# open-mmlab/Live2Diff

Hardware: AMD Instinct MI355X
Metric: frames/sec @512×512, 2 denoise steps; per-step latency; 1/2/4/8 GPU (higher is better)
Workload: dtype f16; 1 GPU; BASELINE configs[1]: 512x512 image (64x64 latent), 2 denoise steps, KV window L=16 (8 sink + 8 rolling), SD-1.5 UNet widths + Live2Diff temporal attention, one independent stream per GPU; plan_launches=433, hipgraph=False, device=AMD Radeon Graphics (gfx950:sramecc+:xnack-, 256 CUs), output_finite=True, default_workload=True

## Files before the change

### live2diff_amd/csrc/flash_attn.hip

```cpp
#include "common.h"

struct FAArgs {
    const h16 *q, *k, *vt;
    h16 *out;
    int B, H, d, Tq, Tk, ldq, ldk, ldvt, ldo;
    long long sq, sk, svt, so;
};

template <int D>
struct FACfg {
    static constexpr int DQK = ((D + 31) / 32) * 32;
    static constexpr int KK = DQK / 32;
    static constexpr int D16 = (D + 15) / 16;
    static constexpr int KROW = DQK + 16;
    static constexpr int VROW = 72;
    static constexpr int KCH = (64 * (DQK / 8)) / 256;
    static constexpr int VTOT = D16 * 16 * 8;
    static constexpr int VCH = (VTOT + 255) / 256;
    static constexpr int TILE_HALFS = 64 * KROW + D16 * 16 * VROW;
    static constexpr int NBUF = (TILE_HALFS * 2 * 2 <= 65536) ? 2 : 1;
    static constexpr bool ONES = (D % 16) != 0;
};

template <int D>
// ... 114 lines not shown
                mx = fmaxf(fmaxf(mx, fmaxf(sacc[ks][qs][0], sacc[ks][qs][1])), fmaxf(sacc[ks][qs][2], sacc[ks][qs][3]));
            mx = fmaxf(mx, __shfl_xor(mx, 16, 64));
            mx = fmaxf(mx, __shfl_xor(mx, 32, 64));
            if (__any((mx - mrow[qs]) * c2e > 8.0f)) {
                const float mnew = fmaxf(mrow[qs], mx);
                const float alpha = __builtin_amdgcn_exp2f((mrow[qs] - mnew) * c2e);
                mrow[qs] = mnew;
                lrow[qs] *= alpha;
#pragma unroll
                for (int ds = 0; ds < D16; ++ds) oacc[ds][qs] *= alpha;
            }
            const float mneg = -mrow[qs] * c2e;
            float psum = 0.f;
#pragma unroll
            for (int ks = 0; ks < 4; ++ks)
#pragma unroll
                for (int r = 0; r < 4; ++r) {
                    const float pv = __builtin_amdgcn_exp2f(fmaf(sacc[ks][qs][r], c2e, mneg));
                    if (!Cf::ONES) psum += pv;
                    pf[ks >> 1][qs][(ks & 1) * 4 + r] = (h16)pv;
                }
            if (!Cf::ONES) lrow[qs] += psum;
        }
#pragma unroll
        for (int c2 = 0; c2 < 2; ++c2)
#pragma unroll
            for (int ds = 0; ds < D16; ++ds) {
                const h16 *vr = Vs + (ds * 16 + li) * VROW + c2 * 32 + lg * 4;
                h16x4 lo = *reinterpret_cast<const h16x4 *>(vr);
                h16x4 hi = *reinterpret_cast<const h16x4 *>(vr + 16);
                h16x8 vf = __builtin_shufflevector(lo, hi, 0, 1, 2, 3, 4, 5, 6, 7);
#pragma unroll
                for (int qs = 0; qs < 2; ++qs)
                    oacc[ds][qs] = __builtin_amdgcn_mfma_f32_16x16x32_f16(vf, pf[c2][qs], oacc[ds][qs], 0, 0, 0);
            }
        if (NBUF == 2) {
            if (kt + 1 < nt) store_tiles(cur ^ 1);
            __syncthreads();
            cur ^= 1;
        } else {
            __syncthreads();
            if (kt + 1 < nt) store_tiles(0);
            __syncthreads();
        }
    }
#pragma unroll
    for (int qs = 0; qs < 2; ++qs) {
        float l;
        if (Cf::ONES) {
            l = __shfl(oacc[D / 16][qs][D % 4], ((D % 16) / 4) * 16 + li, 64);
        } else {
            l = lrow[qs];
            l += __shfl_xor(l, 16, 64);
            l += __shfl_xor(l, 32, 64);
        }
        const float inv = 1.0f / l;
        const int qr = q0 + qs * 16 + li;
        if (qr >= a.Tq) continue;
#pragma unroll
        for (int ds = 0; ds < D16; ++ds) {
            int dc = ds * 16 + lg * 4;
            if (dc >= D) continue;
            h16x4 o;
#pragma unroll
            for (int r = 0; r < 4; ++r) o[r] = (h16)(oacc[ds][qs][r] * inv);
            *reinterpret_cast<h16x4 *>(op + (long long)qr * a.ldo + dc) = o;
        }
    }
}

template <int D>
__global__ __launch_bounds__(256) void flash_attn_kernel(FAArgs a) { flash_attn_body<D>(a); }
template <int D>
__global__ __launch_bounds__(256) __attribute__((amdgpu_waves_per_eu(2))) void flash_attn_kernel_w2(FAArgs a) { flash_attn_body<D>(a); }

template <int D>
static void launch_fa(const FAArgs &a, hipStream_t s) {
    dim3 grid((a.Tq + 127) / 128, a.H, a.B);
    if (D <= 80) hipLaunchKernelGGL((flash_attn_kernel_w2<D>), grid, dim3(256), 0, s, a);
    else hipLaunchKernelGGL((flash_attn_kernel<D>), grid, dim3(256), 0, s, a);
}

int l2d_launch_flash_ring(const l2d_op *op, int qs, hipStream_t s);

int l2d_launch_flash_attn(const l2d_op *op, hipStream_t s) {
    FAArgs a;
    a.q = (const h16 *)op->p[0]; a.k = (const h16 *)op->p[1]; a.vt = (const h16 *)op->p[2]; a.out = (h16 *)op->p[3];
    a.B = op->i[0]; a.H = op->i[1]; a.d = op->i[2]; a.Tq = op->i[3]; a.Tk = op->i[4];
    a.ldq = op->i[5]; a.ldk = op->i[6]; a.ldvt = op->i[7]; a.ldo = op->i[8];
    a.sq = op->l[0]; a.sk = op->l[1]; a.svt = op->l[2]; a.so = op->l[3];
    if (!a.q || !a.k || !a.vt || !a.out || a.B <= 0 || a.H <= 0 || a.Tq <= 0 || a.Tk <= 0 || (a.ldq % 8) || (a.ldk % 8) ||
        (a.ldvt % 8) || (a.ldo % 4) || a.ldvt < ((a.Tk + 7) / 8) * 8) {
        l2d_set_error("flash_attn(tag %d): invalid arguments (B=%d H=%d d=%d Tq=%d Tk=%d ldvt=%d)", op->tag, a.B, a.H, a.d,
                      a.Tq, a.Tk, a.ldvt);
        return L2D_EINVAL;
    }
    const int variant = op->i[9];
    if (variant < 0 || variant > 4) {
        l2d_set_error("flash_attn(tag %d): unknown variant %d", op->tag, variant);
        return L2D_EINVAL;
    }
    const bool ring_ok = op->p[4] && (a.d % 8) == 0 && ((((uintptr_t)a.k) | ((uintptr_t)a.vt)) & 15) == 0 &&
                         ((a.sk | a.svt) % 8) == 0;
    if (variant >= 2 && !ring_ok) {
        l2d_set_error("flash_attn(tag %d): ring variant needs p4 = zero page, d %% 8 == 0 and 16-byte aligned K / V^T", op->tag);
        return L2D_EINVAL;
    }
    L2D_DRY_RETURN();
    if (variant != 1 && ring_ok) {
        int rc = l2d_launch_flash_ring(op, variant >= 2 ? variant : 0, s);
        if (rc != L2D_OK) {
            l2d_set_error("flash_attn(tag %d): unsupported head dim %d (built: 8,16,32,40,64,80,160)", op->tag, a.d);
            return rc;
        }
        return l2d_check_launch("flash_attn_ring", op->tag);
    }
    switch (a.d) {
        case 8: launch_fa<8>(a, s); break;
        case 16: launch_fa<16>(a, s); break;
        case 32: launch_fa<32>(a, s); break;
        case 40: launch_fa<40>(a, s); break;
        case 64: launch_fa<64>(a, s); break;
        case 80: launch_fa<80>(a, s); break;
        case 160: launch_fa<160>(a, s); break;
        default:
            l2d_set_error("flash_attn(tag %d): unsupported head dim %d (built: 8,16,32,40,64,80,160)", op->tag, a.d);
            return L2D_EINVAL;
    }
    return l2d_check_launch("flash_attn", op->tag);
}
```

### live2diff_amd/csrc/tattn.hip

```cpp
#include "tattn.h"

__device__ __forceinline__ float dot8(h16x8 a, h16x8 b) {
    float s = 0.f;
#pragma unroll
    for (int e = 0; e < 8; ++e) s += (float)a[e] * (float)b[e];
    return s;
}

template <int TP, int PB, int L, bool PV = true, int ABL = 0>
__global__ __launch_bounds__(TP *PB) void tattn_stream_kernel(TAttnArgs a) {
    constexpr int HG = TP / 8;
    constexpr int LP = L + 4;
    constexpr bool PRELOAD_V = PV && (L <= 24);
    extern __shared__ __attribute__((aligned(16))) float sp[];

    const int tid = threadIdx.x;
    const int p = tid / TP, cc = tid - p * TP;
    const long long NT = (long long)a.N * a.T;
    const long long pix = (long long)blockIdx.x * PB + p;
    const bool valid = pix < NT;
    const int n = valid ? (int)(pix / a.T) : 0;
    const long long t = valid ? pix - (long long)n * a.T : 0;
    const int C = a.C;
    const int u = (int)a.update_idx[n];
// ... 337 lines not shown
    int v = a.variant;
    if (v == 0) v = (L <= 16) ? 1 : 2;
    if (v == 1 && L <= 16)
        hipLaunchKernelGGL((tattn_stream_kernel<TP, PB, (L <= 16 ? L : 16)>), dim3(nb), dim3(TP * PB), lds, s, a);
#ifdef L2D_PROBES
    else if (v == 8 && L <= 16)
        hipLaunchKernelGGL((tattn_stream_kernel<TP, PB, (L <= 16 ? L : 16), true, 1>), dim3(nb), dim3(TP * PB), lds, s, a);
    else if (v == 9 && L <= 16)
        hipLaunchKernelGGL((tattn_stream_kernel<TP, PB, (L <= 16 ? L : 16), true, 2>), dim3(nb), dim3(TP * PB), lds, s, a);
    else if (v >= 10 && v <= 12 && L <= 16) {
        constexpr int LL = (L <= 16 ? L : 16);
        if (v == 10) hipLaunchKernelGGL((tattn_probe_kernel<TP, PB, LL, 0>), dim3(nb), dim3(TP * PB), 0, s, a);
        if (v == 11) hipLaunchKernelGGL((tattn_probe_kernel<TP, PB, LL, 1>), dim3(nb), dim3(TP * PB), 0, s, a);
        if (v == 12) hipLaunchKernelGGL((tattn_probe_kernel<TP, PB, LL, 2>), dim3(nb), dim3(TP * PB), 0, s, a);
    }
#else
    else if (v >= 8 && v <= 12) {
        l2d_set_error("tattn_stream: variants 8-12 are analysis probes (output is not attention); build with `make PROBES=1`");
        return L2D_EINVAL;
    }
#endif
    else if (v == 7 && L <= 16)
        hipLaunchKernelGGL((tattn_stream_lds_kernel<TP, PB, (L <= 16 ? L : 16)>), dim3(nb), dim3(TP * PB),
                           lds + (size_t)2 * L * TP * 8 * sizeof(h16), s, a);
    else if (v == 5 && L <= 16)
        hipLaunchKernelGGL((tattn_stream_kernel<TP, PB, (L <= 16 ? L : 16), false>), dim3(nb), dim3(TP * PB), lds, s, a);
    else if (v == 6 && L <= 16 && PB >= 2) {
        constexpr int PB2 = PB >= 2 ? PB / 2 : 1;
        int nb2 = (int)((NT + PB2 - 1) / PB2);
        hipLaunchKernelGGL((tattn_stream_kernel<TP, PB2, (L <= 16 ? L : 16)>), dim3(nb2), dim3(TP * PB2),
                           (size_t)TP * PB2 * (L + 4) * sizeof(float), s, a);
    }
    else if (v == 3)
        hipLaunchKernelGGL((tattn_stream_chunked_kernel<TP, PB, L, 4>), dim3(nb), dim3(TP * PB), lds, s, a);
    else if (v == 4 && L % 16 == 0)
        hipLaunchKernelGGL((tattn_stream_chunked_kernel<TP, PB, L, (L % 16 == 0 ? 16 : 4)>), dim3(nb), dim3(TP * PB), lds, s, a);
    else
        hipLaunchKernelGGL((tattn_stream_chunked_kernel<TP, PB, L, (L % 8 == 0 ? 8 : 4)>), dim3(nb), dim3(TP * PB), lds, s, a);
    return L2D_OK;
}

template <int TP, int PB>
static int launch_stream_l(const TAttnArgs &a, hipStream_t s) {
    switch (a.L) {
        case 12: return launch_stream_t<TP, PB, 12>(a, s);
        case 16: return launch_stream_t<TP, PB, 16>(a, s);
        case 24: return launch_stream_t<TP, PB, 24>(a, s);
        case 40: return launch_stream_t<TP, PB, 40>(a, s);
    }
    l2d_set_error("tattn_stream: unsupported window L=%d (built: 12,16,24,40)", a.L);
    return L2D_EINVAL;
}

static int tattn_common(const l2d_op *op, TAttnArgs &a, const char *what) {
    a.qkv = (const h16 *)op->p[0]; a.cache = (h16 *)op->p[1];
    a.q_pe = (const h16 *)op->p[2]; a.k_pe = (const h16 *)op->p[3]; a.v_pe = (const h16 *)op->p[4];
    a.pe_idx = (const long long *)op->p[5]; a.update_idx = (const long long *)op->p[6];
    a.bias = (const h16 *)op->p[7]; a.out = (h16 *)op->p[8];
    a.N = op->i[0]; a.T = op->i[1]; a.C = op->i[2]; a.L = op->i[3]; a.H = op->i[4]; a.variant = op->i[5];
#ifdef L2D_PROBES
    {
        extern unsigned long long *l2d_tattn_probe_ptr();
        a.probe = l2d_tattn_probe_ptr();
    }
#endif
    if (!a.qkv || !a.cache || !a.q_pe || !a.k_pe || !a.v_pe || !a.out || a.N <= 0 || a.T <= 0 || a.H != 8 ||
        (a.C % 64) || a.L <= 0) {
        l2d_set_error("%s(tag %d): invalid arguments (N=%d T=%d C=%d L=%d H=%d; need H=8, C%%64==0)", what, op->tag, a.N,
                      a.T, a.C, a.L, a.H);
        return L2D_EINVAL;
    }
    return L2D_OK;
}

int l2d_launch_tattn_stream(const l2d_op *op, hipStream_t s) {
    TAttnArgs a;
    int rc = tattn_common(op, a, "tattn_stream");
    if (rc) return rc;
    if (!a.pe_idx || !a.update_idx || !a.bias) {
        l2d_set_error("tattn_stream(tag %d): pe_idx/update_idx/bias missing", op->tag);
        return L2D_EINVAL;
    }
    L2D_DRY_RETURN();
    if (a.variant == 13 || (a.variant == 0 && l2d_tattn_ring_ok(a, op->p[9]))) {
        if (!l2d_tattn_ring_ok(a, op->p[9])) {
            l2d_set_error("tattn_stream(tag %d): ring variant needs C in {320,640,1280}, L in {12,16,24,40}, T %% 8 == 0, p9 = zero page", op->tag);
            return L2D_EINVAL;
        }
        rc = l2d_launch_tattn_ring(a, op->p[9], s);
        if (rc) return rc;
        return l2d_check_launch("tattn_stream_ring", op->tag);
    }
    switch (a.C) {
        case 64: rc = launch_stream_l<8, 32>(a, s); break;
        case 128: rc = launch_stream_l<16, 16>(a, s); break;
        case 256: rc = launch_stream_l<32, 8>(a, s); break;
        case 320: rc = launch_stream_l<40, 8>(a, s); break;
        case 640: rc = launch_stream_l<80, 4>(a, s); break;
        case 1280: rc = launch_stream_l<160, 2>(a, s); break;
        default:
            l2d_set_error("tattn_stream(tag %d): unsupported C=%d (built: 64,128,256,320,640,1280)", op->tag, a.C);
            return L2D_EINVAL;
    }
    if (rc) return rc;
    return l2d_check_launch("tattn_stream", op->tag);
}

template <int TP, int PB, int F>
__global__ __launch_bounds__(TP *PB) void tattn_warmup_kernel(TAttnArgs a) {
    constexpr int HG = TP / 8;
    constexpr int LP = F * F + 4;
    extern __shared__ __attribute__((aligned(16))) float sp[];
    const int tid = threadIdx.x;
    const int p = tid / TP, cc = tid - p * TP;
    const long long t = (long long)blockIdx.x * PB + p;
    const bool valid = t < a.T;
    const int C = a.C, L = a.L;
    h16x8 q[F], k[F], v[F];
#pragma unroll
    for (int f = 0; f < F; ++f) {
        q[f] = k[f] = v[f] = l2d_zero8();
        if (valid) {
            const h16 *src = a.qkv + ((long long)f * a.T + t) * 3 * C + cc * 8;
            q[f] = l2d_ld8(src);
            k[f] = l2d_ld8(src + C);
            v[f] = l2d_ld8(src + 2 * C);
            l2d_st8(a.cache + ((0LL * a.T + t) * L + f) * C + cc * 8, k[f]);
            l2d_st8(a.cache + ((1LL * a.T + t) * L + f) * C + cc * 8, v[f]);
        }
        q[f] = q[f] + l2d_ld8(a.q_pe + (long long)f * C + cc * 8);
        k[f] = k[f] + l2d_ld8(a.k_pe + (long long)f * C + cc * 8);
        v[f] = v[f] + l2d_ld8(a.v_pe + (long long)f * C + cc * 8);
    }
    float *row = sp + (long long)tid * LP;
#pragma unroll
    for (int fq = 0; fq < F; ++fq)
#pragma unroll
        for (int fk = 0; fk < F; fk += 4)
            *reinterpret_cast<f32x4 *>(row + fq * F + fk) =
                (f32x4){dot8(q[fq], k[fk]), dot8(q[fq], k[fk + 1]), dot8(q[fq], k[fk + 2]), dot8(q[fq], k[fk + 3])};
    __syncthreads();
    const int gs = p * TP + (cc / HG) * HG;
    const float scale = rsqrtf((float)(C / a.H));
#pragma unroll
    for (int fq = 0; fq < F; ++fq) {
        float s[F];
#pragma unroll
        for (int fk = 0; fk < F; ++fk) s[fk] = 0.f;
        for (int j = 0; j < HG; ++j) {
            const float *r = sp + (long long)(gs + j) * LP + fq * F;
#pragma unroll
            for (int fk = 0; fk < F; fk += 4) {
                f32x4 x = *reinterpret_cast<const f32x4 *>(r + fk);
                s[fk] += x[0]; s[fk + 1] += x[1]; s[fk + 2] += x[2]; s[fk + 3] += x[3];
            }
        }
        float mx = -3.0e38f;
#pragma unroll
        for (int fk = 0; fk < F; ++fk) { s[fk] *= scale; mx = fmaxf(mx, s[fk]); }
        float den = 0.f;
#pragma unroll
        for (int fk = 0; fk < F; ++fk) { s[fk] = __expf(s[fk] - mx); den += s[fk]; }
        const float inv = 1.0f / den;
        float o[8];
#pragma unroll
        for (int e = 0; e < 8; ++e) o[e] = 0.f;
#pragma unroll
// ... 48 lines not shown
```

### live2diff_amd/csrc/tattn_ring.hip

```cpp
#include <stdlib.h>

#include "tattn.h"

#define L2D_GPTR(p) ((__attribute__((address_space(1))) const void *)(p))
#define L2D_LPTR(p) ((__attribute__((address_space(3))) void *)(p))

typedef unsigned int u32x4 __attribute__((ext_vector_type(4)));

#ifdef L2D_PROBES
static unsigned long long *g_tattn_probe = nullptr;
extern "C" void l2d_tattn_set_probe(void *p) { g_tattn_probe = (unsigned long long *)p; }
unsigned long long *l2d_tattn_probe_ptr() { return g_tattn_probe; }
#define TR_STAMP(gi, s, i)                                                                                          \
    do {                                                                                                            \
        if (a.probe && (gi) == 1 && ((s) == 1 || (s) == NSTG / 2 + 1) && (threadIdx.x & 63) == 0)                    \
            a.probe[(((unsigned long long)blockIdx.x * 16 + (threadIdx.x >> 6)) * 2 + ((s) == 1 ? 0 : 1)) * 8 + (i)] = \
                __builtin_readcyclecounter();                                                                       \
    } while (0)
#else
#define TR_STAMP(gi, s, i) do { } while (0)
#endif

__device__ __forceinline__ float ring_dot8(h16x8 a, h16x8 b) {
    float s = 0.f;
// ... 106 lines not shown
        h16x8 q8 = qn;
        if (gi == 0) q8 = l2d_ld8(qkv_b + qoff);
        q8 = q8 + qpe;
        h16 *ku = kbase + (long long)gi * (PB * L * C) + u * C;
        float sc[L];
        float o[8];
#pragma unroll
        for (int e = 0; e < 8; ++e) o[e] = 0.f;
#pragma unroll
        for (int s = 0; s < NSTG; ++s) {
            TR_STAMP(gi, s, 0);
            if (total - 1 - it >= NS - 2) asm volatile("s_waitcnt vmcnt(%0) lgkmcnt(0)" ::"n"((NS - 2) * LPS) : "memory");
            else asm volatile("s_waitcnt vmcnt(0) lgkmcnt(0)" ::: "memory");
            TR_STAMP(gi, s, 1);
            __builtin_amdgcn_s_barrier();
            TR_STAMP(gi, s, 2);
            const bool refill = it_issue < total;
            if (refill) issue();
            TR_STAMP(gi, s, 3);
            const h16 *st = ring + cs_slot * STAGE_H + tid * 8;
            if (s < NSTG / 2) {
#pragma unroll
                for (int r = 0; r < R; ++r) {
                    const int l = s * R + r;
                    h16x8 kk = l2d_ld8(st + r * NT * 8);
                    if (l == u) l2d_st8(ku + coff, kk);
                    kk = kk + l2d_ld8(kpt + l * 320);
                    sc[l] = ring_dot8(q8, kk);
                }
                if (s == NSTG / 2 - 1) {
#pragma unroll
                    for (int l = 0; l < L; l += 4) *reinterpret_cast<f32x4 *>(row + l) = (f32x4){sc[l], sc[l + 1], sc[l + 2], sc[l + 3]};
                    asm volatile("s_waitcnt lgkmcnt(0)" ::: "memory");
                    __builtin_amdgcn_s_barrier();
#pragma unroll
                    for (int l = 0; l < L; ++l) sc[l] = 0.f;
#pragma unroll 2
                    for (int j = 0; j < HG; ++j) {
                        const float *rr = sp + (gs + j) * LP;
#pragma unroll
                        for (int l = 0; l < L; l += 4) {
                            f32x4 x = *reinterpret_cast<const f32x4 *>(rr + l);
                            sc[l] += x[0]; sc[l + 1] += x[1]; sc[l + 2] += x[2]; sc[l + 3] += x[3];
                        }
                    }
                    float mx = -3.0e38f;
#pragma unroll
                    for (int l = 0; l < L; l += 4) {
                        const f32x4 b4 = *reinterpret_cast<const f32x4 *>(blds + l);
#pragma unroll
                        for (int e = 0; e < 4; ++e) { sc[l + e] = sc[l + e] * scale + b4[e]; mx = fmaxf(mx, sc[l + e]); }
                    }
                    float den = 0.f;
#pragma unroll
                    for (int l = 0; l < L; ++l) { sc[l] = __expf(sc[l] - mx); den += sc[l]; }
                    const float inv = 1.0f / den;
#pragma unroll
                    for (int l = 0; l < L; ++l) sc[l] *= inv;
                }
            } else {
                if (s == NSTG / 2 && gi + 1 < ng)
                    qn = l2d_ld8(qkv_b + (long long)(gi + 1) * (PB * 3 * C) + qoff);
#pragma unroll
                for (int r = 0; r < R; ++r) {
                    const int l = (s - NSTG / 2) * R + r;
                    h16x8 vv = l2d_ld8(st + r * NT * 8);
                    if (l == u) l2d_st8(ku + slab + coff, vv);
                    vv = vv + l2d_ld8(vpt + l * 320);
                    ring_axpy8(o, sc[l], vv);
                }
            }
            TR_STAMP(gi, s, 4);
            ++it;
            cs_slot = (cs_slot + 1 == NS) ? 0 : cs_slot + 1;
        }
        h16x8 ov;
#pragma unroll
        for (int e = 0; e < 8; ++e) ov[e] = (h16)o[e];
        l2d_st8(out_b + (long long)gi * (PB * C) + ooff, ov);
    }
}
#endif

template <int HG, int L, int R, int NS>
__global__ __launch_bounds__(384) void tattn_stream_ringlw_kernel(TAttnArgs a, const h16 *zero, int gpb, int groups_per_unit) {
    constexpr int PB = 8, TP = 40, NT = TP * PB, NSTG = 2 * L / R, LPSL = 5 * R;
    constexpr int STAGE_H = R * PB * TP * 8;
    constexpr int LP = L + 4;
    static_assert((NS - 2) * LPSL < 64 && L % 4 == 0 && L % R == 0, "geometry");
    extern __shared__ __attribute__((aligned(16))) unsigned char ring_raw[];
    h16 *ring = reinterpret_cast<h16 *>(ring_raw);
    float *sp = reinterpret_cast<float *>(ring_raw + (size_t)NS * STAGE_H * sizeof(h16));
    float *blds = sp + NT * LP;
    h16 *kpl = reinterpret_cast<h16 *>(blds + L);
    h16 *vpl = kpl + L * 320;

    const int tid = threadIdx.x;
    const int wave = __builtin_amdgcn_readfirstlane(tid >> 6);
    const int C = a.C, CH = C / 320;
    const int bpu = (groups_per_unit + gpb - 1) / gpb;
    const int unit = __builtin_amdgcn_readfirstlane(blockIdx.x / bpu);
    const int n = __builtin_amdgcn_readfirstlane(unit / CH);
    const int chunk = unit - n * CH;
    const int g0 = (blockIdx.x - unit * bpu) * gpb;
    const int ng = min(gpb, groups_per_unit - g0);
    const long long slab = (long long)a.T * L * C;
    h16 *kbase = a.cache + (long long)n * 2 * slab + (long long)g0 * PB * L * C + chunk * 320;
    h16 *vbase = kbase + slab;
    const h16 *qkv_b = a.qkv + ((long long)n * a.T + g0 * PB) * 3 * C + chunk * 320;
    h16 *out_b = a.out + ((long long)n * a.T + g0 * PB) * C + chunk * 320;
    const int u = __builtin_amdgcn_readfirstlane((int)a.update_idx[n]);
    const long long *pei = a.pe_idx + (long long)n * L;
    const h16 *bi = a.bias + (long long)n * L;
    const int total = ng * NSTG;

    if (wave == 5) {
        const int lane = tid & 63;
        unsigned long long live = 0;
        for (int l = 0; l < L; ++l)
            if ((float)bi[l] > -1e30f && l != u) live |= 1ull << l;
        live = ((unsigned long long)(unsigned)__builtin_amdgcn_readfirstlane((int)(live >> 32)) << 32) |
               (unsigned)__builtin_amdgcn_readfirstlane((int)(live & 0xffffffffull));
        unsigned coff[5], qoff[5];
#pragma unroll
        for (int k = 0; k < 5; ++k) {
            const int v = k * 64 + lane, p = v / TP, cc = v - p * TP;
            coff[k] = (unsigned)(p * L * C + cc * 8);
            qoff[k] = (unsigned)(p * 3 * C + cc * 8);
        }
        int it_issue = 0, is_s = 0, is_slot = 0, is_g = 0;
        auto issue = [&]() {
            const bool isv = is_s >= NSTG / 2;
            const int l0 = (isv ? is_s - NSTG / 2 : is_s) * R;
            const h16 *cb = (isv ? vbase : kbase) + (long long)is_g * (PB * L * C);
            const h16 *qb = qkv_b + (long long)is_g * (PB * 3 * C) + (isv ? 2 * C : C);
            h16 *dst = ring + is_slot * STAGE_H;
#pragma unroll
            for (int j = 0; j < R; ++j) {
                const int l = l0 + j;
                const unsigned long long lv = 0ull - ((live >> l) & 1ull);
                const unsigned long long nw = (0ull - (unsigned long long)(l == u ? 1u : 0u)) & ~lv;
                const unsigned long long sb = ((unsigned long long)(cb + l * C) & lv) | ((unsigned long long)qb & nw) |
                                              ((unsigned long long)zero & ~(lv | nw));
#pragma unroll
                for (int k = 0; k < 5; ++k) {
                    const unsigned vo = (coff[k] & (unsigned)lv) | (qoff[k] & (unsigned)nw);
                    __builtin_amdgcn_global_load_lds(L2D_GPTR(reinterpret_cast<const h16 *>(sb) + vo), L2D_LPTR(dst + j * NT * 8 + k * 512), 16, 0, 0);
                }
            }
            ++it_issue;
            if (++is_s == NSTG) { is_s = 0; ++is_g; }
            is_slot = (is_slot + 1 == NS) ? 0 : is_slot + 1;
        };
#pragma unroll
        for (int s = 0; s < NS - 1; ++s)
            if (it_issue < total) issue();
        int it = 0;
        for (int gi = 0; gi < ng; ++gi) {
#pragma unroll 1
            for (int s = 0; s < NSTG; ++s) {
                TR_STAMP(gi, s, 0);
                if (total - 1 - it >= NS - 2) asm volatile("s_waitcnt vmcnt(%0)" ::"n"((NS - 2) * LPSL) : "memory");
                else asm volatile("s_waitcnt vmcnt(0)" ::: "memory");
                TR_STAMP(gi, s, 1);
                __builtin_amdgcn_s_barrier();
                TR_STAMP(gi, s, 2);
                if (it_issue < total) issue();
                TR_STAMP(gi, s, 3);
                TR_STAMP(gi, s, 4);
                if (s == NSTG / 2 - 1) {
                    __builtin_amdgcn_s_barrier();
                    __builtin_amdgcn_s_barrier();
                }
                ++it;
            }
        }
        return;
    }

    const int p = tid / TP, cc = tid - p * TP;
    const unsigned coff = (unsigned)(p * L * C + cc * 8);
    const unsigned qoff = (unsigned)(p * 3 * C + cc * 8);
    const unsigned ooff = (unsigned)(p * C + cc * 8);
    if (tid < L) blds[tid] = (float)bi[tid];
    for (int f0 = 0; f0 < L * TP; f0 += NT) {
        const int f = f0 + tid;
        if (f < L * TP) {
            const int l = f / TP, c = f - l * TP;
            const long long po = pei[l] * C + chunk * 320 + c * 8;
            __builtin_amdgcn_global_load_lds(L2D_GPTR(a.k_pe + po), L2D_LPTR(kpl + (f0 + wave * 64) * 8), 16, 0, 0);
            __builtin_amdgcn_global_load_lds(L2D_GPTR(a.v_pe + po), L2D_LPTR(vpl + (f0 + wave * 64) * 8), 16, 0, 0);
        }
    }
    const h16x8 qpe = l2d_ld8(a.q_pe + pei[u] * C + chunk * 320 + cc * 8);
    h16x8 qn = l2d_ld8(qkv_b + qoff);
    asm volatile("s_waitcnt vmcnt(0)" ::: "memory");

    const float scale = rsqrtf((float)(C / a.H));
    const int gs = p * TP + (cc / HG) * HG;
    float *row = sp + tid * LP;
    const h16 *kpt = kpl + cc * 8, *vpt = vpl + cc * 8;
    int cs_slot = 0;
    for (int gi = 0; gi < ng; ++gi) {
        const h16x8 q8 = qn + qpe;
        h16 *ku = kbase + (long long)gi * (PB * L * C) + u * C;
#pragma unroll 1
        for (int s = 0; s < NSTG / 2; ++s) {
            TR_STAMP(gi, s, 0);
            asm volatile("s_waitcnt lgkmcnt(0)" ::: "memory");
            TR_STAMP(gi, s, 1);
            __builtin_amdgcn_s_barrier();
            TR_STAMP(gi, s, 2);
            TR_STAMP(gi, s, 3);
            const h16 *st = ring + cs_slot * STAGE_H + tid * 8;
            float d[R];
#pragma unroll
            for (int r = 0; r < R; ++r) {
                const int l = s * R + r;
                h16x8 kk = l2d_ld8(st + r * NT * 8);
                if (l == u) l2d_st8(ku + coff, kk);
                kk = kk + l2d_ld8(kpt + l * 320);
                d[r] = ring_dot8(q8, kk);
            }
            if constexpr (R == 2) *reinterpret_cast<f32x2 *>(row + s * 2) = (f32x2){d[0], d[1]};
            else {
#pragma unroll
                for (int r = 0; r < R; ++r) row[s * R + r] = d[r];
            }
            TR_STAMP(gi, s, 4);
            cs_slot = (cs_slot + 1 == NS) ? 0 : cs_slot + 1;
        }
        asm volatile("s_waitcnt lgkmcnt(0)" ::: "memory");
        __builtin_amdgcn_s_barrier();
        float sc[L];
#pragma unroll
        for (int l = 0; l < L; ++l) sc[l] = 0.f;
#pragma unroll 2
        for (int j = 0; j < HG; ++j) {
            const float *rr = sp + (gs + j) * LP;
#pragma unroll
            for (int l = 0; l < L; l += 4) {
                const f32x4 x = *reinterpret_cast<const f32x4 *>(rr + l);
                sc[l] += x[0]; sc[l + 1] += x[1]; sc[l + 2] += x[2]; sc[l + 3] += x[3];
            }
        }
        float mx = -3.0e38f;
#pragma unroll
        for (int l = 0; l < L; l += 4) {
            const f32x4 b4 = *reinterpret_cast<const f32x4 *>(blds + l);
#pragma unroll
            for (int e = 0; e < 4; ++e) { sc[l + e] = sc[l + e] * scale + b4[e]; mx = fmaxf(mx, sc[l + e]); }
        }
        float den = 0.f;
#pragma unroll
        for (int l = 0; l < L; ++l) { sc[l] = __expf(sc[l] - mx); den += sc[l]; }
        const float inv = 1.0f / den;
        asm volatile("s_waitcnt lgkmcnt(0)" ::: "memory");
        __builtin_amdgcn_s_barrier();
#pragma unroll
        for (int l = 0; l < L; l += 4) *reinterpret_cast<f32x4 *>(row + l) = (f32x4){sc[l] * inv, sc[l + 1] * inv, sc[l + 2] * inv, sc[l + 3] * inv};
        if (gi + 1 < ng) qn = l2d_ld8(qkv_b + (long long)(gi + 1) * (PB * 3 * C) + qoff);
        float o[8];
#pragma unroll
        for (int e = 0; e < 8; ++e) o[e] = 0.f;
#pragma unroll 1
        for (int s = 0; s < NSTG / 2; ++s) {
            TR_STAMP(gi, s + NSTG / 2, 0);
            asm volatile("s_waitcnt lgkmcnt(0)" ::: "memory");
            TR_STAMP(gi, s + NSTG / 2, 1);
            __builtin_amdgcn_s_barrier();
            TR_STAMP(gi, s + NSTG / 2, 2);
            TR_STAMP(gi, s + NSTG / 2, 3);
            const h16 *st = ring + cs_slot * STAGE_H + tid * 8;
            float pr[R];
            if constexpr (R == 2) { const f32x2 t = *reinterpret_cast<const f32x2 *>(row + s * 2); pr[0] = t[0]; pr[1] = t[1]; }
            else {
#pragma unroll
                for (int r = 0; r < R; ++r) pr[r] = row[s * R + r];
            }
#pragma unroll
            for (int r = 0; r < R; ++r) {
                const int l = s * R + r;
                h16x8 vv = l2d_ld8(st + r * NT * 8);
                if (l == u) l2d_st8(ku + slab + coff, vv);
                vv = vv + l2d_ld8(vpt + l * 320);
                ring_axpy8(o, pr[r], vv);
            }
            TR_STAMP(gi, s + NSTG / 2, 4);
            cs_slot = (cs_slot + 1 == NS) ? 0 : cs_slot + 1;
        }
        h16x8 ov;
#pragma unroll
        for (int e = 0; e < 8; ++e) ov[e] = (h16)o[e];
        l2d_st8(out_b + (long long)gi * (PB * C) + ooff, ov);
    }
}

template <int L, int HG, int R, int NS>
static void launch_ringlw(const TAttnArgs &a, const h16 *zero, int slots, hipStream_t s) {
    constexpr int NT = 320;
    constexpr size_t LDS = (size_t)NS * R * 8 * 40 * 16 + (size_t)(NT * (L + 4) + L) * sizeof(float) + (size_t)2 * L * 320 * sizeof(h16);
    static_assert(LDS <= 160 * 1024, "tattn ring geometry exceeds the CU's LDS");
    static bool attr_done_dev[L2D_MAX_DEV] = {false};
    bool &attr_done = attr_done_dev[l2d_dev_ordinal()];
    if (!attr_done) {
        if (hipFuncSetAttribute((const void *)tattn_stream_ringlw_kernel<HG, L, R, NS>, hipFuncAttributeMaxDynamicSharedMemorySize, (int)LDS) == hipSuccess)
            attr_done = true;
        else
            (void)hipGetLastError();
    }
    const int CH = a.C / 320;
    const int groups_per_unit = a.T / 8;
    const int total = a.N * CH * groups_per_unit;
    const int gpb = (total + slots - 1) / slots;
    const int bpu = (groups_per_unit + gpb - 1) / gpb;
    hipLaunchKernelGGL((tattn_stream_ringlw_kernel<HG, L, R, NS>), dim3(a.N * CH * bpu), dim3(384), LDS, s, a, zero, gpb, groups_per_unit);
}

#ifdef L2D_PROBES
template <int L, int HG, int R, int NS, int PB>
static void launch_ring_g(const TAttnArgs &a, const h16 *zero, int slots, hipStream_t s) {
    constexpr int NT = 40 * PB;
    constexpr size_t LDS = (size_t)NS * R * PB * 40 * 16 + (size_t)(NT * (L + 4) + L) * sizeof(float) + (size_t)2 * L * 320 * sizeof(h16);
    static_assert(LDS <= 160 * 1024, "tattn ring geometry exceeds the CU's LDS");
    static bool attr_done_dev[L2D_MAX_DEV] = {false};
    bool &attr_done = attr_done_dev[l2d_dev_ordinal()];
    if (!attr_done) {
        if (hipFuncSetAttribute((const void *)tattn_stream_ring_kernel<HG, L, R, NS, PB>, hipFuncAttributeMaxDynamicSharedMemorySize, (int)LDS) == hipSuccess)
            attr_done = true;
        else
            (void)hipGetLastError();
    }
    const int CH = a.C / 320;
    const int groups_per_unit = a.T / PB;
    const int total = a.N * CH * groups_per_unit;
    const int gpb = (total + slots - 1) / slots;
    const int bpu = (groups_per_unit + gpb - 1) / gpb;
    hipLaunchKernelGGL((tattn_stream_ring_kernel<HG, L, R, NS, PB>), dim3(a.N * CH * bpu), dim3(NT), LDS, s, a, zero, gpb, groups_per_unit);
}
#endif

template <int L, int HG>
static void launch_ring(const TAttnArgs &a, const h16 *zero, int cus, hipStream_t s) {
#ifdef L2D_PROBES
    static int geo = -2;
    if (geo == -2) {
        const char *e = getenv("L2D_TATTN_RING");
        geo = e ? atoi(e) : -1;
    }
    if constexpr (L <= 16) { if (geo == 4) { launch_ring_g<L, HG, 4, 5, 8>(a, zero, cus, s); return; } }
    else if constexpr (L == 24) { if (geo == 4) { launch_ring_g<L, HG, 4, 4, 8>(a, zero, cus, s); return; } }
#endif
    if constexpr (L <= 16) {
        launch_ringlw<L, HG, 4, 5>(a, zero, cus, s);
    } else if constexpr (L == 24) {
        launch_ringlw<L, HG, 4, 4>(a, zero, cus, s);
    } else {
        launch_ringlw<L, HG, 2, 5>(a, zero, cus, s);
    }
}

bool l2d_tattn_ring_ok(const TAttnArgs &a, const void *zero) {
    return zero && (a.C == 320 || a.C == 640 || a.C == 1280) && (a.L == 16 || a.L == 12 || a.L == 24 || a.L == 40) && (a.T % 8 == 0) && a.H == 8;
}

int l2d_launch_tattn_ring(const TAttnArgs &a, const void *zero_page, hipStream_t s) {
    static int cus = 0;
    if (!cus) {
        int dev = 0;
        hipDeviceProp_t prop;
        if (hipGetDevice(&dev) != hipSuccess || hipGetDeviceProperties(&prop, dev) != hipSuccess) return L2D_ELAUNCH;
        cus = prop.multiProcessorCount > 0 ? prop.multiProcessorCount : 256;
    }
    const h16 *zero = (const h16 *)zero_page;
    if (a.L == 16) {
        if (a.C == 320) launch_ring<16, 5>(a, zero, cus, s);
        else if (a.C == 640) launch_ring<16, 10>(a, zero, cus, s);
        else launch_ring<16, 20>(a, zero, cus, s);
    } else if (a.L == 12) {
        if (a.C == 320) launch_ring<12, 5>(a, zero, cus, s);
        else if (a.C == 640) launch_ring<12, 10>(a, zero, cus, s);
        else launch_ring<12, 20>(a, zero, cus, s);
    } else if (a.L == 24) {
        if (a.C == 320) launch_ring<24, 5>(a, zero, cus, s);
        else if (a.C == 640) launch_ring<24, 10>(a, zero, cus, s);
        else launch_ring<24, 20>(a, zero, cus, s);
    } else {
        if (a.C == 320) launch_ring<40, 5>(a, zero, cus, s);
        else if (a.C == 640) launch_ring<40, 10>(a, zero, cus, s);
        else launch_ring<40, 20>(a, zero, cus, s);
    }
    return L2D_OK;
}
```

Baseline: 133.5 frames/s.

## Add short-key flash attention kernel and narrow temporal-attention ring for small grids

Adds a single-pass flash attention kernel for cross-attention with at most 128 keys (d=40/80/160). It loads all K/V tiles into LDS at once, computes the softmax without an online rescale, and picks waves per block from the tile count. It is auto-selected when the tile count is small relative to CU count. Separately, the temporal-attention ring kernel is generalised to a pixel-block size parameter, and a narrow PB=2 variant is launched when the work would otherwise underfill the CUs. Together these aim to raise occupancy and cut per-tile overhead on small launches, at the cost of more code paths and masked-lane handling.

Result: no change. 134.2 frames/s (median of 6 runs) (+0.6%).

```diff
diff --git a/live2diff_amd/csrc/flash_attn.hip b/live2diff_amd/csrc/flash_attn.hip
--- a/live2diff_amd/csrc/flash_attn.hip
+++ b/live2diff_amd/csrc/flash_attn.hip
@@ -220,6 +220,9 @@
 }
 
 int l2d_launch_flash_ring(const l2d_op *op, int qs, hipStream_t s);
+int l2d_launch_flash_short(const l2d_op *op, hipStream_t s);
+bool l2d_flash_short_ok(int d, int Tk);
+bool l2d_flash_short_auto(const l2d_op *op);
 
 int l2d_launch_flash_attn(const l2d_op *op, hipStream_t s) {
     FAArgs a;
@@ -234,7 +237,7 @@
         return L2D_EINVAL;
     }
     const int variant = op->i[9];
-    if (variant < 0 || variant > 4) {
+    if (variant < 0 || variant > 5) {
         l2d_set_error("flash_attn(tag %d): unknown variant %d", op->tag, variant);
         return L2D_EINVAL;
     }
@@ -244,7 +247,19 @@
         l2d_set_error("flash_attn(tag %d): ring variant needs p4 = zero page, d %% 8 == 0 and 16-byte aligned K / V^T", op->tag);
         return L2D_EINVAL;
     }
+    if (variant == 5 && !l2d_flash_short_ok(a.d, a.Tk)) {
+        l2d_set_error("flash_attn(tag %d): the short-key variant covers Tk <= 128 and d = 40 / 80 / 160 (Tk=%d d=%d)", op->tag, a.Tk, a.d);
+        return L2D_EINVAL;
+    }
     L2D_DRY_RETURN();
+    if (variant == 5 || (variant == 0 && ring_ok && l2d_flash_short_auto(op))) {
+        int rc = l2d_launch_flash_short(op, s);
+        if (rc != L2D_OK) {
+            l2d_set_error("flash_attn(tag %d): short-key launch failed", op->tag);
+            return rc;
+        }
+        return l2d_check_launch("flash_attn_short", op->tag);
+    }
     if (variant != 1 && ring_ok) {
         int rc = l2d_launch_flash_ring(op, variant >= 2 ? variant : 0, s);
         if (rc != L2D_OK) {
diff --git a/live2diff_amd/csrc/flash_attn_short.hip b/live2diff_amd/csrc/flash_attn_short.hip
--- /dev/null
+++ b/live2diff_amd/csrc/flash_attn_short.hip
@@ -0,0 +1,273 @@
+#include "common.h"
+
+#define L2D_GPTR(p) ((__attribute__((address_space(1))) const void *)(p))
+#define L2D_LPTR(p) ((__attribute__((address_space(3))) void *)(p))
+
+struct FASArgs {
+    const h16 *q, *k, *vt, *zero;
+    h16 *out;
+    int B, H, Tq, Tk, ldq, ldk, ldvt, ldo;
+    long long sq, sk, svt, so;
+};
+
+__device__ __forceinline__ float fas_row_max(float v) {
+    auto r = __builtin_amdgcn_permlane16_swap(__float_as_uint(v), __float_as_uint(v), false, false);
+    v = fmaxf(__uint_as_float(r[0]), __uint_as_float(r[1]));
+    r = __builtin_amdgcn_permlane32_swap(__float_as_uint(v), __float_as_uint(v), false, false);
+    return fmaxf(__uint_as_float(r[0]), __uint_as_float(r[1]));
+}
+
+template <int D>
+struct FASCfg {
+    static constexpr int KK = (D + 31) / 32;
+    static constexpr int D16 = (D + 15) / 16;
+    static constexpr int DV = D16 * 16;
+    static constexpr bool ONES = (D % 16) != 0;
+    static constexpr int KBYTES = KK * 64 * 32 * 2;
+    static constexpr int VBYTES = DV * 64 * 2;
+    static constexpr int TILE = KBYTES + VBYTES;
+    static constexpr int NKI = KK * 4;
+    static constexpr int NVI = D / 8;
+};
+
+template <int D, int NW>
+__global__ __launch_bounds__(64 * NW) void flash_shortkey_kernel(FASArgs a) {
+    using Cf = FASCfg<D>;
+    static_assert(D % 8 == 0, "head size: whole 16-byte pieces");
+    constexpr int KK = Cf::KK, D16 = Cf::D16, DV = Cf::DV, NKI = Cf::NKI, NVI = Cf::NVI, NT = 64 * NW;
+    constexpr int TILE_H = Cf::TILE / 2, KH = Cf::KBYTES / 2;
+    extern __shared__ __attribute__((aligned(16))) h16 smem[];
+
+    const int tid = threadIdx.x, lane = tid & 63;
+    const int wave = __builtin_amdgcn_readfirstlane(tid >> 6);
+    const int li = lane & 15, lg = lane >> 4;
+    const int nqb = (a.Tq + 16 * NW - 1) / (16 * NW);
+    int wgid;
+    {
+        const int nwg = gridDim.x, q = nwg >> 3, r = nwg & 7, xcd = blockIdx.x & 7, idx = blockIdx.x >> 3;
+        wgid = (xcd < r ? xcd * (q + 1) : r * (q + 1) + (xcd - r) * q) + idx;
+    }
+    const int bh = wgid / nqb, qb = wgid - bh * nqb;
+    const int b = bh / a.H, h = bh - b * a.H;
+    const int q0 = qb * (16 * NW) + wave * 16;
+    const h16 *qp = a.q + (long long)b * a.sq + h * D;
+    const h16 *kp = a.k + (long long)b * a.sk + h * D;
+    const h16 *vp = a.vt + (long long)b * a.svt + (long long)h * D * a.ldvt;
+    h16 *op = a.out + (long long)b * a.so + h * D;
+    const int Tk = a.Tk;
+    const int nt = (Tk + 63) >> 6;
+
+    h16x8 qraw[KK];
+#pragma unroll
+    for (int kk = 0; kk < KK; ++kk) {
+        const int qr = min(q0 + li, a.Tq - 1), dc = kk * 32 + lg * 8;
+        qraw[kk] = l2d_ld8(qp + (long long)qr * a.ldq + (dc < D ? dc : 0));
+    }
+    __builtin_amdgcn_sched_barrier(0);
+
+    {
+        const int r16 = lane >> 2;
+        const int kcol = (((lane & 3) ^ ((r16 >> 1) & 3)) << 3);
+        const int kkey = ((r16 >> 2) << 3) | (r16 & 3);
+        const h16 *kp0 = kp + (long long)kkey * a.ldk + kcol;
+        const int vkey0 = (((lane & 7) ^ (lane >> 4)) << 3);
+        const h16 *vp0 = vp + (long long)(lane >> 3) * a.ldvt;
+#pragma unroll
+        for (int kt = 0; kt < 2; ++kt) {
+            if (kt < nt) {
+                h16 *st = smem + kt * TILE_H;
+#pragma unroll
+                for (int g = 0; g < 4; ++g) {
+                    const int gkey = kt * 64 + (g >> 1) * 32 + (g & 1) * 4;
+                    if ((g % NW) == wave && gkey < Tk) {
+                        const bool live = gkey + kkey < Tk;
+                        const h16 *rp = live ? kp0 + (long long)gkey * a.ldk : a.zero;
+                        const int kstep = live ? 32 : 0;
+#pragma unroll
+                        for (int kk = 0; kk < KK; ++kk) {
+                            const h16 *src = rp + kk * kstep;
+                            if ((kk + 1) * 32 > D) src = (kk * 32 + kcol < D) ? src : a.zero;
+                            __builtin_amdgcn_global_load_lds(L2D_GPTR(src), L2D_LPTR(st + kk * 2048 + g * 512), 16, 0, 0);
+                        }
+                    }
+                }
+                const h16 *vb[2];
+                long long vstep[2];
+#pragma unroll
+                for (int par = 0; par < 2; ++par) {
+                    const int key = kt * 64 + (vkey0 ^ (par * 32));
+                    vb[par] = key < Tk ? vp0 + key : a.zero;
+                    vstep[par] = key < Tk ? 8ll * a.ldvt : 0ll;
+                }
+#pragma unroll
+                for (int j = 0; j < NVI; ++j)
+                    if ((j % NW) == wave)
+                        __builtin_amdgcn_global_load_lds(L2D_GPTR(vb[j & 1] + j * vstep[j & 1]), L2D_LPTR(st + KH + j * 512), 16, 0, 0);
+            }
+        }
+    }
+
+    if (Cf::ONES) {
+        h16x8 one;
+#pragma unroll
+        for (int e = 0; e < 8; ++e) one[e] = (h16)1.0f;
+        for (int i = tid; i < nt * (DV - D) * 8; i += NT) {
+            const int kt = i / ((DV - D) * 8), r = (i / 8) % (DV - D), sl = i & 7;
+            l2d_st8(smem + kt * TILE_H + KH + (D + r) * 64 + sl * 8, r == 0 ? one : l2d_zero8());
+        }
+    }
+
+    const float c2e = rsqrtf((float)D) * 1.4426950408889634f;
+    h16x8 qf[KK];
+    {
+        h16x8 sc;
+#pragma unroll
+        for (int e = 0; e < 8; ++e) sc[e] = (h16)c2e;
+#pragma unroll
+        for (int kk = 0; kk < KK; ++kk) {
+            const int qr = q0 + li, dc = kk * 32 + lg * 8;
+            qf[kk] = (qr < a.Tq && dc < D) ? qraw[kk] * sc : l2d_zero8();
+        }
+    }
+
+    asm volatile("s_waitcnt vmcnt(0)" ::: "memory");
+    __syncthreads();
+    if (Tk & 7) {
+        const int first = Tk & 63, last = ((Tk + 7) & ~7) & 63;
+        h16 *vs = smem + (nt - 1) * TILE_H + KH;
+        for (int r = tid; r < D; r += NT) {
+            const int sw = (r >> 1) & 7;
+            for (int c = first; c < (last == 0 ? 64 : last); ++c) vs[r * 64 + ((((c >> 3) ^ sw)) << 3) + (c & 7)] = (h16)0.0f;
+        }
+        __syncthreads();
+    }
+
+    const int kswz = (li >> 1) & 3, vswz = (li >> 1) & 7;
+    const int koff = li * 32 + ((lg ^ kswz) << 3);
+    f32x4 S[8];
+#pragma unroll
+    for (int kt = 0; kt < 2; ++kt)
+#pragma unroll
+        for (int ks = 0; ks < 4; ++ks) {
+            const int gkey = kt * 64 + (ks >> 1) * 32 + (ks & 1) * 4;
+            f32x4 acc = (f32x4){0.f, 0.f, 0.f, 0.f};
+            if (gkey < Tk) {
+                const h16 *st = smem + kt * TILE_H;
+#pragma unroll
+                for (int kk = 0; kk < KK; ++kk)
+                    acc = __builtin_amdgcn_mfma_f32_16x16x32_f16(l2d_ld8(st + kk * 2048 + ks * 512 + koff), qf[kk], acc, 0, 0, 0);
+            }
+#pragma unroll
+            for (int r = 0; r < 4; ++r) S[kt * 4 + ks][r] = (gkey + lg * 8 + r < Tk) ? acc[r] : -3.0e38f;
+        }
+
+    float m = fmaxf(fmaxf(S[0][0], S[0][1]), fmaxf(S[0][2], S[0][3]));
+#pragma unroll
+    for (int i = 1; i < 8; ++i) m = fmaxf(fmaxf(m, fmaxf(S[i][0], S[i][1])), fmaxf(S[i][2], S[i][3]));
+    m = fas_row_max(m);
+    h16x8 pf[4];
+    float psum = 0.f;
+#pragma unroll
+    for (int i = 0; i < 8; ++i)
+#pragma unroll
+        for (int r = 0; r < 4; ++r) {
+            const float pv = __builtin_amdgcn_exp2f(S[i][r] - m);
+            if (!Cf::ONES) psum += pv;
+            pf[i >> 1][(i & 1) * 4 + r] = (h16)pv;
+        }
+
+    f32x4 oacc[D16];
+#pragma unroll
+    for (int ds = 0; ds < D16; ++ds) oacc[ds] = (f32x4){0.f, 0.f, 0.f, 0.f};
+#pragma unroll
+    for (int c = 0; c < 4; ++c) {
+        if (c * 32 < Tk) {
+            const h16 *st = smem + (c >> 1) * TILE_H + KH + li * 64 + ((((c & 1) * 4 + lg) ^ vswz) << 3);
+#pragma unroll
+            for (int ds = 0; ds < D16; ++ds)
+                oacc[ds] = __builtin_amdgcn_mfma_f32_16x16x32_f16(l2d_ld8(st + ds * 1024), pf[c], oacc[ds], 0, 0, 0);
+        }
+    }
+
+    float l;
+    if (Cf::ONES) {
+        l = __shfl(oacc[D / 16][D % 4], ((D % 16) / 4) * 16 + li, 64);
+    } else {
+        l = psum;
+        l += __shfl_xor(l, 16, 64);
+        l += __shfl_xor(l, 32, 64);
+    }
+    const float inv = 1.0f / l;
+    const int qr = q0 + li;
+    if (qr >= a.Tq) return;
+#pragma unroll
+    for (int ds = 0; ds < D16; ++ds) {
+        const int dc = ds * 16 + lg * 4;
+        if (dc >= D) continue;
+        h16x4 o;
+#pragma unroll
+        for (int r = 0; r < 4; ++r) o[r] = (h16)(oacc[ds][r] * inv);
+        *reinterpret_cast<h16x4 *>(op + (long long)qr * a.ldo + dc) = o;
+    }
+}
+
+template <int D, int NW>
+static void launch_fas_w(const FASArgs &a, hipStream_t s) {
+    using Cf = FASCfg<D>;
+    const int nt = (a.Tk + 63) / 64;
+    const size_t lds = (size_t)nt * Cf::TILE;
+    static bool attr_done_dev[L2D_MAX_DEV] = {false};
+    bool &attr_done = attr_done_dev[l2d_dev_ordinal()];
+    if (2 * Cf::TILE > 65536 && !attr_done) {
+        if (hipFuncSetAttribute((const void *)flash_shortkey_kernel<D, NW>, hipFuncAttributeMaxDynamicSharedMemorySize, 2 * Cf::TILE) == hipSuccess)
+            attr_done = true;
+        else
+            (void)hipGetLastError();
+    }
+    dim3 grid(((a.Tq + 16 * NW - 1) / (16 * NW)) * a.H * a.B);
+    hipLaunchKernelGGL((flash_shortkey_kernel<D, NW>), grid, dim3(64 * NW), lds, s, a);
+}
+
+template <int D>
+static void launch_fas(const FASArgs &a, int cus, hipStream_t s) {
+    const long long tiles = (long long)((a.Tq + 15) / 16) * a.H * a.B;
+    if (tiles <= cus) launch_fas_w<D, 1>(a, s);
+    else if (tiles < 4ll * cus) launch_fas_w<D, 2>(a, s);
+    else launch_fas_w<D, 4>(a, s);
+}
+
+bool l2d_flash_short_ok(int d, int Tk) { return Tk >= 1 && Tk <= 128 && (d == 40 || d == 80 || d == 160); }
+
+static int fas_cus() {
+    static int cus = 0;
+    if (!cus) {
+        int dev = 0;
+        hipDeviceProp_t prop;
+        if (hipGetDevice(&dev) != hipSuccess || hipGetDeviceProperties(&prop, dev) != hipSuccess) return 0;
+        cus = prop.multiProcessorCount > 0 ? prop.multiProcessorCount : 256;
+    }
+    return cus;
+}
+
+bool l2d_flash_short_auto(const l2d_op *op) {
+    const long long tiles = (long long)((op->i[3] + 15) / 16) * op->i[1] * op->i[0];
+    return l2d_flash_short_ok(op->i[2], op->i[4]) && tiles <= 4ll * fas_cus();
+}
+
+int l2d_launch_flash_short(const l2d_op *op, hipStream_t s) {
+    const int cus = fas_cus();
+    if (!cus) return L2D_ELAUNCH;
+    FASArgs a;
+    a.q = (const h16 *)op->p[0]; a.k = (const h16 *)op->p[1]; a.vt = (const h16 *)op->p[2]; a.out = (h16 *)op->p[3];
+    a.zero = (const h16 *)op->p[4];
+    a.B = op->i[0]; a.H = op->i[1]; a.Tq = op->i[3]; a.Tk = op->i[4];
+    a.ldq = op->i[5]; a.ldk = op->i[6]; a.ldvt = op->i[7]; a.ldo = op->i[8];
+    a.sq = op->l[0]; a.sk = op->l[1]; a.svt = op->l[2]; a.so = op->l[3];
+    if (!l2d_flash_short_ok(op->i[2], a.Tk)) return L2D_EINVAL;
+    switch (op->i[2]) {
+        case 40: launch_fas<40>(a, cus, s); break;
+        case 80: launch_fas<80>(a, cus, s); break;
+        default: launch_fas<160>(a, cus, s); break;
+    }
+    return L2D_OK;
+}
diff --git a/live2diff_amd/csrc/tattn.hip b/live2diff_amd/csrc/tattn.hip
--- a/live2diff_amd/csrc/tattn.hip
+++ b/live2diff_amd/csrc/tattn.hip
@@ -443,7 +443,7 @@
         return L2D_EINVAL;
     }
     L2D_DRY_RETURN();
-    if (a.variant == 13 || (a.variant == 0 && l2d_tattn_ring_ok(a, op->p[9]))) {
+    if (a.variant == 13 || a.variant == 14 || (a.variant == 0 && l2d_tattn_ring_ok(a, op->p[9]))) {
         if (!l2d_tattn_ring_ok(a, op->p[9])) {
             l2d_set_error("tattn_stream(tag %d): ring variant needs C in {320,640,1280}, L in {12,16,24,40}, T %% 8 == 0, p9 = zero page", op->tag);
             return L2D_EINVAL;
diff --git a/live2diff_amd/csrc/tattn_ring.hip b/live2diff_amd/csrc/tattn_ring.hip
--- a/live2diff_amd/csrc/tattn_ring.hip
+++ b/live2diff_amd/csrc/tattn_ring.hip
@@ -212,9 +212,10 @@
 }
 #endif
 
-template <int HG, int L, int R, int NS>
-__global__ __launch_bounds__(384) void tattn_stream_ringlw_kernel(TAttnArgs a, const h16 *zero, int gpb, int groups_per_unit) {
-    constexpr int PB = 8, TP = 40, NT = TP * PB, NSTG = 2 * L / R, LPSL = 5 * R;
+template <int HG, int L, int R, int NS, int PB>
+__device__ __forceinline__ void tattn_ringlw_body(const TAttnArgs &a, const h16 *zero, int gpb, int groups_per_unit) {
+    constexpr int TP = 40, NT = TP * PB, NCW = (NT + 63) / 64, NSTG = 2 * L / R, LPSL = NCW * R;
+    constexpr bool FULL = (NT % 64) == 0;
     constexpr int STAGE_H = R * PB * TP * 8;
     constexpr int LP = L + 4;
     static_assert((NS - 2) * LPSL < 64 && L % 4 == 0 && L % R == 0, "geometry");
@@ -244,17 +245,17 @@
     const h16 *bi = a.bias + (long long)n * L;
     const int total = ng * NSTG;
 
-    if (wave == 5) {
+    if (wave == NCW) {
         const int lane = tid & 63;
         unsigned long long live = 0;
         for (int l = 0; l < L; ++l)
             if ((float)bi[l] > -1e30f && l != u) live |= 1ull << l;
         live = ((unsigned long long)(unsigned)__builtin_amdgcn_readfirstlane((int)(live >> 32)) << 32) |
                (unsigned)__builtin_amdgcn_readfirstlane((int)(live & 0xffffffffull));
-        unsigned coff[5], qoff[5];
-#pragma unroll
-        for (int k = 0; k < 5; ++k) {
-            const int v = k * 64 + lane, p = v / TP, cc = v - p * TP;
+        unsigned coff[NCW], qoff[NCW];
+#pragma unroll
+        for (int k = 0; k < NCW; ++k) {
+            const int v = min(k * 64 + lane, NT - 1), p = v / TP, cc = v - p * TP;
             coff[k] = (unsigned)(p * L * C + cc * 8);
             qoff[k] = (unsigned)(p * 3 * C + cc * 8);
         }
@@ -273,9 +274,10 @@
                 const unsigned long long sb = ((unsigned long long)(cb + l * C) & lv) | ((unsigned long long)qb & nw) |
                                               ((unsigned long long)zero & ~(lv | nw));
 #pragma unroll
-                for (int k = 0; k < 5; ++k) {
+                for (int k = 0; k < NCW; ++k) {
                     const unsigned vo = (coff[k] & (unsigned)lv) | (qoff[k] & (unsigned)nw);
-                    __builtin_amdgcn_global_load_lds(L2D_GPTR(reinterpret_cast<const h16 *>(sb) + vo), L2D_LPTR(dst + j * NT * 8 + k * 512), 16, 0, 0);
+                    if (FULL || k < NCW - 1 || lane < NT - (NCW - 1) * 64)
+                        __builtin_amdgcn_global_load_lds(L2D_GPTR(reinterpret_cast<const h16 *>(sb) + vo), L2D_LPTR(dst + j * NT * 8 + k * 512), 16, 0, 0);
                 }
             }
             ++it_issue;
@@ -308,14 +310,16 @@
         return;
     }
 
-    const int p = tid / TP, cc = tid - p * TP;
+    const bool act = FULL || tid < NT;
+    const int wi = FULL ? tid : min(tid, NT - 1);
+    const int p = wi / TP, cc = wi - p * TP;
     const unsigned coff = (unsigned)(p * L * C + cc * 8);
     const unsigned qoff = (unsigned)(p * 3 * C + cc * 8);
     const unsigned ooff = (unsigned)(p * C + cc * 8);
     if (tid < L) blds[tid] = (float)bi[tid];
     for (int f0 = 0; f0 < L * TP; f0 += NT) {
         const int f = f0 + tid;
-        if (f < L * TP) {
+        if (act && f < L * TP) {
             const int l = f / TP, c = f - l * TP;
             const long long po = pei[l] * C + chunk * 320 + c * 8;
             __builtin_amdgcn_global_load_lds(L2D_GPTR(a.k_pe + po), L2D_LPTR(kpl + (f0 + wave * 64) * 8), 16, 0, 0);
@@ -328,7 +332,7 @@
 
     const float scale = rsqrtf((float)(C / a.H));
     const int gs = p * TP + (cc / HG) * HG;
-    float *row = sp + tid * LP;
+    float *row = sp + wi * LP;
     const h16 *kpt = kpl + cc * 8, *vpt = vpl + cc * 8;
     int cs_slot = 0;
     for (int gi = 0; gi < ng; ++gi) {
@@ -342,20 +346,22 @@
             __builtin_amdgcn_s_barrier();
             TR_STAMP(gi, s, 2);
             TR_STAMP(gi, s, 3);
-            const h16 *st = ring + cs_slot * STAGE_H + tid * 8;
+            const h16 *st = ring + cs_slot * STAGE_H + wi * 8;
             float d[R];
 #pragma unroll
             for (int r = 0; r < R; ++r) {
                 const int l = s * R + r;
                 h16x8 kk = l2d_ld8(st + r * NT * 8);
-                if (l == u) l2d_st8(ku + coff, kk);
+                if (l == u && act) l2d_st8(ku + coff, kk);
                 kk = kk + l2d_ld8(kpt + l * 320);
                 d[r] = ring_dot8(q8, kk);
             }
-            if constexpr (R == 2) *reinterpret_cast<f32x2 *>(row + s * 2) = (f32x2){d[0], d[1]};
-            else {
-#pragma unroll
-                for (int r = 0; r < R; ++r) row[s * R + r] = d[r];
+            if (act) {
+                if constexpr (R == 2) *reinterpret_cast<f32x2 *>(row + s * 2) = (f32x2){d[0], d[1]};
+                else {
+#pragma unroll
+                    for (int r = 0; r < R; ++r) row[s * R + r] = d[r];
+                }
             }
             TR_STAMP(gi, s, 4);
             cs_slot = (cs_slot + 1 == NS) ? 0 : cs_slot + 1;
@@ -388,7 +394,8 @@
         asm volatile("s_waitcnt lgkmcnt(0)" ::: "memory");
         __builtin_amdgcn_s_barrier();
 #pragma unroll
-        for (int l = 0; l < L; l += 4) *reinterpret_cast<f32x4 *>(row + l) = (f32x4){sc[l] * inv, sc[l + 1] * inv, sc[l + 2] * inv, sc[l + 3] * inv};
+        for (int l = 0; l < L; l += 4)
+            if (act) *reinterpret_cast<f32x4 *>(row + l) = (f32x4){sc[l] * inv, sc[l + 1] * inv, sc[l + 2] * inv, sc[l + 3] * inv};
         if (gi + 1 < ng) qn = l2d_ld8(qkv_b + (long long)(gi + 1) * (PB * 3 * C) + qoff);
         float o[8];
 #pragma unroll
@@ -401,7 +408,7 @@
             __builtin_amdgcn_s_barrier();
             TR_STAMP(gi, s + NSTG / 2, 2);
             TR_STAMP(gi, s + NSTG / 2, 3);
-            const h16 *st = ring + cs_slot * STAGE_H + tid * 8;
+            const h16 *st = ring + cs_slot * STAGE_H + wi * 8;
             float pr[R];
             if constexpr (R == 2) { const f32x2 t = *reinterpret_cast<const f32x2 *>(row + s * 2); pr[0] = t[0]; pr[1] = t[1]; }
             else {
@@ -412,7 +419,7 @@
             for (int r = 0; r < R; ++r) {
                 const int l = s * R + r;
                 h16x8 vv = l2d_ld8(st + r * NT * 8);
-                if (l == u) l2d_st8(ku + slab + coff, vv);
+                if (l == u && act) l2d_st8(ku + slab + coff, vv);
                 vv = vv + l2d_ld8(vpt + l * 320);
                 ring_axpy8(o, pr[r], vv);
             }
@@ -422,8 +429,18 @@
         h16x8 ov;
 #pragma unroll
         for (int e = 0; e < 8; ++e) ov[e] = (h16)o[e];
-        l2d_st8(out_b + (long long)gi * (PB * C) + ooff, ov);
-    }
+        if (act) l2d_st8(out_b + (long long)gi * (PB * C) + ooff, ov);
+    }
+}
+
+template <int HG, int L, int R, int NS>
+__global__ __launch_bounds__(384) void tattn_stream_ringlw_kernel(TAttnArgs a, const h16 *zero, int gpb, int groups_per_unit) {
+    tattn_ringlw_body<HG, L, R, NS, 8>(a, zero, gpb, groups_per_unit);
+}
+
+template <int HG, int L, int R, int NS, int PB>
+__global__ __launch_bounds__(((40 * PB + 63) / 64 + 1) * 64) void tattn_stream_narrow_kernel(TAttnArgs a, const h16 *zero, int gpb, int groups_per_unit) {
+    tattn_ringlw_body<HG, L, R, NS, PB>(a, zero, gpb, groups_per_unit);
 }
 
 template <int L, int HG, int R, int NS>
@@ -445,6 +462,27 @@
     const int gpb = (total + slots - 1) / slots;
     const int bpu = (groups_per_unit + gpb - 1) / gpb;
     hipLaunchKernelGGL((tattn_stream_ringlw_kernel<HG, L, R, NS>), dim3(a.N * CH * bpu), dim3(384), LDS, s, a, zero, gpb, groups_per_unit);
+}
+
+template <int L, int HG, int R, int NS, int PB>
+static void launch_narrow(const TAttnArgs &a, const h16 *zero, int slots, hipStream_t s) {
+    constexpr int NT = 40 * PB, NCW = (NT + 63) / 64;
+    constexpr size_t LDS = (size_t)NS * R * PB * 40 * 16 + (size_t)(NT * (L + 4) + L) * sizeof(float) + (size_t)2 * L * 320 * sizeof(h16);
+    static_assert(LDS <= 160 * 1024, "tattn ring geometry exceeds the CU's LDS");
+    static bool attr_done_dev[L2D_MAX_DEV] = {false};
+    bool &attr_done = attr_done_dev[l2d_dev_ordinal()];
+    if (!attr_done) {
+        if (hipFuncSetAttribute((const void *)tattn_stream_narrow_kernel<HG, L, R, NS, PB>, hipFuncAttributeMaxDynamicSharedMemorySize, (int)LDS) == hipSuccess)
+            attr_done = true;
+        else
+            (void)hipGetLastError();
+    }
+    const int CH = a.C / 320;
+    const int groups_per_unit = a.T / PB;
+    const int total = a.N * CH * groups_per_unit;
+    const int gpb = (total + slots - 1) / slots;
+    const int bpu = (groups_per_unit + gpb - 1) / gpb;
+    hipLaunchKernelGGL((tattn_stream_narrow_kernel<HG, L, R, NS, PB>), dim3(a.N * CH * bpu), dim3((NCW + 1) * 64), LDS, s, a, zero, gpb, groups_per_unit);
 }
 
 #ifdef L2D_PROBES
@@ -481,12 +519,16 @@
     if constexpr (L <= 16) { if (geo == 4) { launch_ring_g<L, HG, 4, 5, 8>(a, zero, cus, s); return; } }
     else if constexpr (L == 24) { if (geo == 4) { launch_ring_g<L, HG, 4, 4, 8>(a, zero, cus, s); return; } }
 #endif
+    const bool narrow = a.variant == 14 || (a.variant == 0 && a.N * (a.C / 320) * (a.T / 8) < cus);
     if constexpr (L <= 16) {
-        launch_ringlw<L, HG, 4, 5>(a, zero, cus, s);
+        if (narrow) launch_narrow<L, HG, 4, 5, 2>(a, zero, cus, s);
+        else launch_ringlw<L, HG, 4, 5>(a, zero, cus, s);
     } else if constexpr (L == 24) {
-        launch_ringlw<L, HG, 4, 4>(a, zero, cus, s);
+        if (narrow) launch_narrow<L, HG, 4, 4, 2>(a, zero, cus, s);
+        else launch_ringlw<L, HG, 4, 4>(a, zero, cus, s);
     } else {
-        launch_ringlw<L, HG, 2, 5>(a, zero, cus, s);
+        if (narrow) launch_narrow<L, HG, 2, 5, 2>(a, zero, cus, s);
+        else launch_ringlw<L, HG, 2, 5>(a, zero, cus, s);
     }
 }
 
```
